# grunwaldlab/krisp

Measured on AMD Instinct MI355X. Metric: k-mers/s sorted+intersected at k=28, higher is better.
Workload: dtype u64

## Files before the change

include/krisp_hip.h:

```cpp
#ifndef KRISP_HIP_H
#define KRISP_HIP_H

#include <stddef.h>
#include <stdint.h>

#ifdef __cplusplus
extern "C" {
#endif

typedef struct kr_ctx kr_ctx;

typedef struct { uint64_t prefix, in_mask, out_mask; } kr_cand;

typedef struct { uint64_t key; uint32_t genome; uint32_t count; } kr_record;

enum {
    KR_OK = 0,
    KR_ERR_HIP = -1,
    KR_ERR_PARAM = -2,
    KR_ERR_CAPACITY = -3,
    KR_ERR_STATE = -4,
    KR_ERR_KEY = -5,
    KR_ERR_HOST = -6
};
// ... 188 lines not shown

int64_t kr_render_records(const kr_record* recs, size_t n, int L, int D, int R, const uint32_t* label_of,
                          size_t n_genomes, const char* const* label_text, size_t n_labels, const uint8_t* label_in,
                          int dot, char** csv, size_t* csv_len, char** align, size_t* align_len);
int64_t kr_render_windows(const uint8_t* rows, size_t n, int L, int D, int R, const uint32_t* cand, const uint32_t* genome,
                          const uint32_t* label_of, size_t n_genomes, const char* const* label_text, size_t n_labels,
                          const uint8_t* label_in, int dot, int rna, char** csv, size_t* csv_len, char** align,
                          size_t* align_len);
void    kr_text_free(void* p);

enum { KR_OPT_SLICE_BASES = 1,
       KR_OPT_GENERIC_INTERSECT = 2,
       KR_OPT_ISECT_FORMAT = 3,
       KR_OPT_ABLATE = 4,
       KR_OPT_WIDE_SLOTS = 5,
       KR_OPT_PLACE_TRIES = 7,
       KR_OPT_ISECT_KERNEL = 8,
       KR_OPT_LANES = 9,
       KR_OPT_LAZY_ORDER = 10,
       KR_OPT_COARSE_REST = 11,
       KR_OPT_COARSE_POOL = 12,
       KR_OPT_JOIN2 = 13,
       KR_OPT_COARSE_ONE_STRAND = 14,
       KR_OPT_WIDE_ORDERED = 6 };
int     kr_set_option(kr_ctx*, int option, int64_t value);

int     kr_sync(kr_ctx*);
int     kr_timer_begin(kr_ctx*);
double  kr_timer_end_ms(kr_ctx*);
int     kr_stage_enable(kr_ctx*, int on);
int     kr_stage_select(kr_ctx*, unsigned stage_mask);
int     kr_stage_reset(kr_ctx*);
double  kr_stage_ms(kr_ctx*, int stage);
int64_t kr_stage_launches(kr_ctx*, int stage);

int64_t kr_debug_fetch(kr_ctx*, int genome_id, int what, void* out, size_t cap_bytes);
int64_t kr_debug_inversions(kr_ctx*, int genome_id);
double  kr_debug_localsort(kr_ctx*, int genome_id, int reps, int mode);
double  kr_debug_intersect(kr_ctx*, const int* genome_ids, int n, const uint8_t* is_ingroup, int reps, int mode);
double  kr_debug_copy_gbps(kr_ctx*, size_t bytes, int reps);
const char* kr_debug_copy_which(kr_ctx*);
int     kr_build_experiments(void);
int     kr_debug_lazy(kr_ctx*, int64_t* out8);
int     kr_debug_isect(kr_ctx*, int64_t* out8);
int     kr_debug_scan(kr_ctx*, int64_t* out8);
int     kr_debug_place(kr_ctx*, double* out8);
int     kr_debug_coarse_pool(kr_ctx*, double* out8);
int     kr_debug_coarse_strand(kr_ctx*, int64_t* out8);
int     kr_debug_comm(kr_ctx*, int64_t* out8);
int     kr_debug_comm_probe(kr_ctx*, size_t bytes, int reps, double* out3);
int64_t kr_debug_cands_selfexchange(kr_ctx*, int apply_filter);
int     kr_debug_comm_hang(kr_ctx*);
int64_t kr_debug_budget_left(kr_ctx*);
int     kr_debug_budget_set(kr_ctx*, int64_t left);
int     kr_debug_info(kr_ctx*, int64_t* out8);

#ifdef __cplusplus
}
#endif
#endif
```

krisp_amd/_native.py:

```python
import ctypes
import os

import numpy as np

HERE = os.path.dirname(os.path.abspath(__file__))
LIB_PATH = os.environ.get("KRISP_HIP_LIB") or os.path.join(HERE, "libkrisp_hip.so")

CAND = np.dtype([("prefix", "<u8"), ("in_mask", "<u8"), ("out_mask", "<u8")])
RECORD = np.dtype([("key", "<u8"), ("genome", "<u4"), ("count", "<u4")])
WIDE_HIT = np.dtype([("cand", "<u4"), ("genome", "<u4"), ("pos", "<u4"), ("strand", "<u4")])
LOC_HIT = np.dtype([("group", "<u4"), ("strand", "<u4"), ("pos", "<u8")])
NEAR_HIT = np.dtype([("target", "<u4"), ("strand", "u1"), ("mismatches", "u1"), ("flank_mismatches", "u1"), ("pad", "u1"),
                     ("pos", "<u8")])
PRODUCT_SITE = np.dtype([("pos", "<u8"), ("entry", "<u4"), ("mismatches", "u1"), ("end_mismatches", "u1"),
                         ("pad", "<u2")])
PRODUCT_HIT = np.dtype([("pos", "<u8"), ("length", "<u4"), ("pair", "<u4"), ("strand", "u1"), ("left_mm", "u1"),
                        ("right_mm", "u1"), ("left_end_mm", "u1"), ("right_end_mm", "u1"), ("pad", "u1", (3,))])
DESIGN_RECORD = np.dtype([("found", "<u4"), ("product_size", "<u4"), ("pair_penalty", "<u4"), ("left_start", "<u2"),
                          ("left_len", "<u2"), ("right_start", "<u2"), ("right_len", "<u2"), ("left_tm", "<i4"), ("right_tm", "<i4"),
                          ("left_gc", "<u2"), ("right_gc", "<u2"), ("left_penalty", "<u4"), ("right_penalty", "<u4"),
                          ("left_self_any", "<i4"), ("left_self_end", "<i4"), ("right_self_any", "<i4"),
                          ("right_self_end", "<i4"), ("pair_any", "<i4"), ("pair_end", "<i4")])
DESIGN_RECORD_HP = np.dtype(DESIGN_RECORD.descr + [("left_hairpin", "<i4"), ("right_hairpin", "<i4")])
PANEL_MEMBER = np.dtype([("position", "<u4"), ("cross_any", "<i4"), ("cross_end", "<i4"), ("dropped", "<u4", (2,))])
# ... 1 lines not shown
GUIDE_RECORD = np.dtype([("found", "<u4"), ("strand", "<u4"), ("start", "<u4"), ("min_mismatches", "<u4"),
                         ("sum_mismatches", "<u4"), ("gc", "<u4"), ("candidates", "<u4"), ("pad", "<u4")])
GUIDE_HIT_RAW = np.dtype([("guide", "<u4"), ("strand", "u1"), ("mismatches", "u1"), ("pam", "u1"), ("pad", "u1"), ("pos", "<u8"),
                          ("columns", "<u8")])
ASSAY_HIT_RAW = np.dtype([("pos", "<u8"), ("length", "<u4"), ("pair", "<u4"), ("strand", "u1"), ("left_mm", "u1"), ("right_mm", "u1"),
                          ("left_end_mm", "u1"), ("right_end_mm", "u1"), ("hit_strand", "u1"), ("hit_mismatches", "u1"),
                          ("hit_pam", "u1"), ("hit_pos", "<u8"), ("columns", "<u8"), ("guide", "<u4"), ("hit", "<u4")])
GUIDE_BULGE_HIT_RAW = np.dtype([("guide", "<u4"), ("strand", "u1"), ("mismatches", "u1"), ("pam", "u1"), ("bulge", "i1"),
                                ("pos", "<u8"), ("columns", "<u8"), ("bulge_column", "<u4"), ("length", "<u4")])
WIDE_DICT_LEFT, WIDE_DICT_RIGHT, WIDE_GROUPS, WIDE_HITS, WIDE_COUNTS, WIDE_SLOT_BITS, WIDE_NGROUPS, WIDE_BATCH_USED, WIDE_LOCATED, WIDE_KEYS_LISTED = 0, 1, 2, 3, 4, 5, 6, 7, 8, 9
WIDE_MAX_K = 1024
WIDE_MAX_FLANK = 256
COMM_ID_BYTES = 128

SOFT_MAP, SOFT_OMIT = 0, 1
OPT_SLICE_BASES, OPT_GENERIC_INTERSECT, OPT_ISECT_FORMAT, OPT_ABLATE, OPT_WIDE_SLOTS, OPT_WIDE_ORDERED, OPT_PLACE_TRIES = 1, 2, 3, 4, 5, 6, 7
OPT_ISECT_KERNEL = 8
OPT_LANES = 9
OPT_LAZY_ORDER = 10
OPT_COARSE_REST = 11
OPT_COARSE_POOL = 12
OPT_JOIN2 = 13
OPT_COARSE_ONE_STRAND = 14
ERR_KEY, ERR_HOST = -5, -6
STRANDS_BOTH, STRANDS_FORWARD, STRANDS_CANONICAL = 0, 1, 2
STAGES = ["pack", "hist8", "reduce8", "scatter1", "hist2", "scan2", "scatter2", "chunks", "localsort",
          "fallback", "intersect", "compact", "collect", "merge", "locate"]
STAGE_KERNELS = {"pack": "k_pack", "hist8": "k_hist8 (wide path: k_hist8w, slices: k_hist8k)", "reduce8": "k_reduce8a+k_reduce8b",
                 "scatter1": "k_scatter1p (wide path: k_scatter1w, slices: k_scatter1kp)",
                 "hist2": "k_hist16 (or k_hist2)", "scan2": "k_hist16_off (or k_scan2)", "scatter2": "k_scatter2",
                 "chunks": "k_chunk_table", "localsort": "k_localsort2",
                 "fallback": "k_seg_merge", "intersect": "k_intersect3 (+ k_intersect for oversized items)",
                 "compact": "k_scan+k_publish_reset+k_gather_items",
                 "collect": "k_collect_count+k_tile_sums+k_scan+k_tile_apply+k_publish+k_collect_emit",
                 "merge": "k_cands_flag+k_scan+k_cands_compact", "locate": "k_wide_locate"}

_c = ctypes
_P = _c.c_void_p
SYMBOLS = [
    ("kr_create", _P, [_c.c_int, _c.c_size_t]),
    ("kr_destroy", None, [_P]),
    ("kr_last_error", _c.c_char_p, [_P]),
    ("kr_set_params", _c.c_int, [_P, _c.c_int, _c.c_int, _c.c_int, _c.c_int, _c.c_size_t]),
    ("kr_set_strands", _c.c_int, [_P, _c.c_int]),
    ("kr_genome_upload", _c.c_int, [_P, _c.c_int, _P, _c.c_size_t]),
    ("kr_genome_sort", _c.c_int, [_P, _c.c_int]),
# ... 825 lines not shown
        v = self.lib.kr_debug_copy_gbps(self.ctx, nbytes, reps)
        if v < 0:
            raise KrispHipError("kr_debug_copy_gbps failed")
        return v

    def mem_info(self):
        o = np.zeros(4, dtype=np.int64)
        self._check(self.lib.kr_mem_info(self.ctx, _ptr(o)), "kr_mem_info")
        return dict(avail=int(o[0]), total=int(o[1]), used=int(o[2]), budget=int(o[3]))

    def debug_comm(self):
        o = np.zeros(8, dtype=np.int64)
        self._check(self.lib.kr_debug_comm(self.ctx, _ptr(o)), "kr_debug_comm")
        return dict(syncs=int(o[0]), p2p=int(o[1]), collectives=int(o[2]), exchange_us=int(o[3]), reduces=int(o[4]),
                    message_entries=int(o[5]))

    def debug_place(self):
        o = np.zeros(8, dtype=np.float64)
        self._check(self.lib.kr_debug_place(self.ctx, _ptr(o)), "kr_debug_place")
        return dict(candidates=int(o[0]), taken=int(o[1]), fastest_ms=[round(float(x), 4) for x in o[2:6]],
                    median_ms=round(float(o[6]), 4), slowest_ms=round(float(o[7]), 4))

    def debug_coarse_strand(self):
        o = np.zeros(8, dtype=np.int64)
        self._check(self.lib.kr_debug_coarse_strand(self.ctx, _ptr(o)), "kr_debug_coarse_strand")
        return dict(partitions=int(o[0]), calls=int(o[1]), rounds_forward=int(o[2]), rounds_reverse=int(o[3]),
                    last_forward=int(o[4]), last_reverse=int(o[5]), on=int(o[6]))

    def debug_coarse_pool(self):
        o = np.zeros(8, dtype=np.float64)
        self._check(self.lib.kr_debug_coarse_pool(self.ctx, _ptr(o)), "kr_debug_coarse_pool")
        return dict(total=int(o[0]), free=int(o[1]), held=int(o[2]), partitions=int(o[3]), searches=int(o[4]),
                    held_ms=[round(float(o[5]), 4), round(float(o[6]), 4)], on=int(o[7]))

    def comm_set_timeout(self, seconds):
        self._check(self.lib.kr_comm_set_timeout(self.ctx, int(seconds)), "kr_comm_set_timeout")

    def debug_comm_hang(self):
        return self._check(self.lib.kr_debug_comm_hang(self.ctx), "kr_debug_comm_hang")

    def cands_selfexchange(self, apply_filter=False):
        return self._check(self.lib.kr_debug_cands_selfexchange(self.ctx, 1 if apply_filter else 0), "kr_debug_cands_selfexchange")

    def comm_probe(self, nbytes=64 << 10, reps=50):
        o = np.zeros(3, dtype=np.float64)
        self._check(self.lib.kr_debug_comm_probe(self.ctx, nbytes, reps, _ptr(o)), "kr_debug_comm_probe")
        return dict(allreduce_sync_us=round(float(o[0]), 2), sendrecv_self_sync_us=round(float(o[1]), 2),
                    bcast_sync_us=round(float(o[2]), 2), message_bytes=int(nbytes))

    def copy_which(self):
# ... 11 lines not shown
```

krisp_amd/csrc/h_core.inc:

```
static thread_local std::string g_last_error;

struct DevBuf {
    void* p = nullptr;
    size_t bytes = 0;
};

struct Slice {
    DevBuf keys, off, chunkstart, chunkdesc, ovf;
    u64 nmax = 0;
    u32 nchunks = 0;
    int64_t count = -1;
    int res = -1;
};

struct Genome {
    int id = -1;
    size_t n_bases = 0;
    u64 nwords = 0;
    u64 nmax = 0;
    DevBuf bases, wkeys;
    DevBuf wlcnt;
    bool wlist = false;
    u32 wlcap = 0;
    std::vector<Slice> sl;
// ... 88 lines not shown
    int join2 = 1;
    u32 j2_grid = 0;
    int j2_occ[9] = {0};
    int64_t j2_launches = 0, j2_full = 0;
    bool j2_full_counted = false;
    int64_t isect_ovf_items = 0, isect_refall = 0;
    int i3_last_T = 0, i3_last_mlog = 0, i3_last_tags = 0, i3_last_ua = 0;
    int64_t isect_ua = 0;
    int fuse_anchor = 1;
    u32 i3_ovf_cap = I3_OVF_CAP;
    int isect_fmt = 0;
    int opt_slice_bases = -1;
    hipEvent_t slice_ready[2] = {nullptr, nullptr};
    bool custom_layout = false;
    bool mixed_alphabets = false;
    int lazy_order = 1;
    bool order_wanted = false;
    int64_t lazy_skipped = 0, lazy_ordered = 0, lazy_touch = 0;
    DevBuf touchdesc, touchovf;
    int coarse_rest = 1;
    int64_t coarse_done = 0, coarse_promoted = 0;
    int coarse_one = 1;
    int64_t one_partitions = 0, one_calls = 0, one_rounds[2] = {0, 0}, one_last[2] = {0, 0};
    DevBuf co_ent;
    int coarse_pool = 1;
    struct PoolBuf { DevBuf buf; double ms; hipEvent_t ev; bool wait; };
    std::vector<PoolBuf> cpool_free;
    int cpool_total = 0;
    int64_t cpool_partitions = 0;
    int64_t cpool_searches = 0;
    size_t place_min_bytes = (size_t)256 << 20;
    DevBuf co_state, co_tab;
    u32 co_tcap = CO_TCAP;
    u32 co_hitcap = 0;
    int co_occ = 0;
    u32 co_grid = 0;
    u32 scan_cap = 0;
    int64_t scan_dbg[3] = {0, 0, 0};
    int slice_route = 1;
    typedef std::vector<DevBuf*> Bufs;
    struct Wide {
        bool on = false;
        int L = 0, D = 0, R = 0, k = 0, omit = 0, W = 0, strands = 0;
        struct DictBufs {
            DevBuf keys, idx, slots;
            DevBuf mzT, mzB;
            int ib = 1, sb = 0, mzlen = 0;
            u32 n = 0, mznb = 0;
            bool canon = false;
            u32 nfull = 0;
            void bufs(Bufs& v) { v.insert(v.end(), {&keys, &idx, &slots, &mzT, &mzB}); }
            Dict view() const {
                Dict d{};
                d.keys = (const u64*)keys.p;
                d.idx = (const u32*)idx.p;
                d.slots = sb && slots.p ? (const uint4*)slots.p : nullptr;
                d.ib = ib;
                d.sb = sb;
// ... 424 lines not shown
        g_last_error = "hipSetDevice failed";
        return nullptr;
    }
    kr_ctx* c = new kr_ctx();
    c->device = device;
    c->budget = hbm_budget_bytes;
    {
        const char* e = getenv("KR_DBG");
        c->dbg = e ? (atoi(e) & 32) : 0;
        const char* e2 = getenv("KR_ISECT_FMT");
        c->isect_fmt = e2 ? (atoi(e2) == 1 ? 1 : (atoi(e2) == 2 ? 2 : 0)) : 0;
        const char* e3 = getenv("KR_SLICE_BASES");
        c->opt_slice_bases = e3 ? std::max(0, std::min(4, atoi(e3))) : -1;
        const char* e16 = getenv("KR_FUSE_ANCHOR");
        c->fuse_anchor = e16 ? atoi(e16) != 0 : 1;
        const char* e15 = getenv("KR_LAZY_ORDER");
        c->lazy_order = e15 ? atoi(e15) != 0 : 1;
        const char* e17 = getenv("KR_COARSE_REST");
        c->coarse_rest = e17 ? atoi(e17) != 0 : 1;
        const char* e21 = getenv("KR_COARSE_POOL");
        c->coarse_pool = e21 ? atoi(e21) != 0 : 1;
        const char* e26 = getenv("KR_COARSE_ONE_STRAND");
        c->coarse_one = e26 ? atoi(e26) != 0 : 1;
        const char* e22 = getenv("KR_PLACE_MIN_BYTES");
        if (e22) c->place_min_bytes = (size_t)std::max(0ll, atoll(e22));
        const char* e18 = getenv("KR_COARSE_TCAP");
        if (e18) c->co_tcap = (u32)std::max(1, std::min((int)CO_TCAP, atoi(e18)));
        const char* e19 = getenv("KR_COARSE_HITCAP");
        if (e19) c->co_hitcap = (u32)std::max(1, atoi(e19));
        const char* e20 = getenv("KR_COARSE_GRID");
        if (e20) c->co_grid = (u32)std::max(0, std::min(65536, atoi(e20)));
        const char* e24 = getenv("KR_JOIN2");
        c->join2 = e24 ? atoi(e24) != 0 : 1;
        const char* e25 = getenv("KR_JOIN2_GRID");
        if (e25) c->j2_grid = (u32)std::max(0, std::min(65536, atoi(e25)));
        const char* e23 = getenv("KR_SCAN_GRID");
        if (e23) c->scan_cap = (u32)std::max(0, std::min(65536, atoi(e23)));
        const char* e13 = getenv("KR_SLICE_ROUTE");
        c->slice_route = e13 ? atoi(e13) != 0 : 1;
        const char* e8 = getenv("KR_PLACE_TRIES");
        c->place_tries = e8 ? std::max(1, std::min(16, atoi(e8))) : 8;
        c->place_tries_set = e8 != nullptr;
        const char* e4 = getenv("KR_WIDE_SLOTS");
        c->wide.use_slots = e4 ? atoi(e4) != 0 : true;
        const char* e7 = getenv("KR_WIDE_SHARE");
        c->wide.use_share = e7 ? atoi(e7) != 0 : true;
        const char* e11 = getenv("KR_WIDE_SPECTRUM");
        c->wide.packed_spectrum = e11 ? atoi(e11) != 0 : true;
        const char* e5 = getenv("KR_WIDE_ORDERED");
        c->wide.ordered = e5 ? atoi(e5) != 0 : false;
// ... 186 lines not shown
        c->place_tries = (int)value;
        c->place_tries_set = true;
        return KR_OK;
    case KR_OPT_WIDE_ORDERED:
        if (value != 0 && value != 1) return fail(c, KR_ERR_PARAM, "KR_OPT_WIDE_ORDERED: 0 or 1");
        c->wide.ordered = value != 0;
        return KR_OK;
    case KR_OPT_LAZY_ORDER:
        if (value != 0 && value != 1) return fail(c, KR_ERR_PARAM, "KR_OPT_LAZY_ORDER: 0 or 1");
        c->lazy_order = (int)value;
        return KR_OK;
    case KR_OPT_COARSE_REST:
        if (value != 0 && value != 1) return fail(c, KR_ERR_PARAM, "KR_OPT_COARSE_REST: 0 or 1");
        c->coarse_rest = (int)value;
        return KR_OK;
    case KR_OPT_COARSE_POOL:
        if (value != 0 && value != 1) return fail(c, KR_ERR_PARAM, "KR_OPT_COARSE_POOL: 0 or 1");
        c->coarse_pool = (int)value;
        return KR_OK;
    case KR_OPT_COARSE_ONE_STRAND:
        if (value != 0 && value != 1) return fail(c, KR_ERR_PARAM, "KR_OPT_COARSE_ONE_STRAND: 0 or 1");
        c->coarse_one = (int)value;
        return KR_OK;
    case KR_OPT_JOIN2:
        if (value != 0 && value != 1) return fail(c, KR_ERR_PARAM, "KR_OPT_JOIN2: 0 or 1");
        c->join2 = (int)value;
        return KR_OK;
    case KR_OPT_ABLATE:
#ifdef KR_ABLATE
        c->dbg = (c->dbg & 32) | ((int)value & ~32);
        return KR_OK;
#else
        return fail(c, KR_ERR_PARAM, "KR_OPT_ABLATE needs a -DKR_ABLATE build");
#endif
    default:
        return fail(c, KR_ERR_PARAM, "unknown option %d", option);
    }
}

int kr_set_strands(kr_ctx* c, int mode) {
    if (!c || !c->have_params) return fail(c, KR_ERR_STATE, "kr_set_params first");
    if (mode < KR_STRANDS_BOTH || mode > KR_STRANDS_CANONICAL) return fail(c, KR_ERR_PARAM, "unknown strand mode %d", mode);
    if (c->wide.on && mode == KR_STRANDS_CANONICAL) return fail(c, KR_ERR_PARAM, "the wide path emits both strands or the forward one");
    if (!c->genomes.empty()) return fail(c, KR_ERR_STATE, "kr_set_strands after genomes were uploaded");
    c->g.strands = mode;
    c->wide.strands = mode;
// ... 1127 lines not shown
```

krisp_amd/csrc/h_intersect.inc:

```
static int64_t intersect_once(kr_ctx* c, const int* ids, int n, const uint8_t* is_in, int apply_filter, bool* redo);

static int64_t cands_merge_device(kr_ctx* c, size_t m, int have_other, int apply_filter);

static inline int fmode(const kr_ctx* c, int apply_filter) { return apply_filter ? (c->mixed_alphabets ? 2 : 1) : 0; }

int kr_set_mixed_alphabets(kr_ctx* c, int on) {
    if (!c) return KR_ERR_PARAM;
    c->mixed_alphabets = on != 0;
    return KR_OK;
}

#define KR_MAX_CANDS 0xFFFFFF00ull
static int cands_fit(kr_ctx* c, uint64_t n, const char* who) {
    if (n < KR_MAX_CANDS) return KR_OK;
    return fail(c, KR_ERR_CAPACITY, "%s: a candidate list of %llu entries exceeds the %llu a list may hold (an intersection that "
                "nothing prunes: give both ingroup and outgroup genomes to one call, or fewer genomes per call)", who,
                (unsigned long long)n, (unsigned long long)KR_MAX_CANDS);
}

static int cands_compact_room(kr_ctx* c, u32 n) {
    const size_t nblk = ((size_t)n + 255) / 256;
    int rc;
    if ((rc = ensure(c, c->flags, (size_t)n * 4))) return rc;
    if ((rc = ensure(c, c->blockcnt, (nblk + 2) * 4))) return rc;
// ... 58 lines not shown
    const u32 nC = (u32)nC64, nblk = (nC + 255) / 256;
    const Geom g = slice_geom(c, 0);
    hipStream_t st = c->stream;
    const u32 hitcap = c->co_hitcap ? c->co_hitcap : (u32)std::min<u64>(2ull * nC + 65536, 0x7FFFFFF0ull);
    if ((rc = ensure(c, c->co_state, (size_t)nC * 4))) return rc;
    if ((rc = ensure(c, c->co_tab, (size_t)(2 * 260 + 256 * CO_ROW) * 4))) return rc;
    if ((rc = cands_compact_room(c, nC))) return rc;
    const size_t ent_bytes = (size_t)2 * nC * sizeof(CoEnt);
    if (one && (rc = ensure(c, c->co_ent, ent_bytes + (size_t)(3 * CS_CLS + 8) * 4))) return rc;
    for (Genome* G : cg) {
        if (G->hitcap < hitcap || !G->hits.p) {
            if ((rc = ensure(c, G->hits, (size_t)hitcap * 8 + 16))) return rc;
        }
        G->hitcap = hitcap;
        G->hits_valid = false;
    }
    if (c->co_occ == 0) {
        int per = 0;
        const hipError_t e = hipOccupancyMaxActiveBlocksPerMultiprocessor(&per, k_coarse_probe<0>, CO_T, 0);
        c->co_occ = (e == hipSuccess && per >= 1) ? per : 1;
        if (hipOccupancyMaxActiveBlocksPerMultiprocessor(&per, k_coarse_probe<1>, CO_T, 0) == hipSuccess && per >= 1)
            c->co_occ = std::min(c->co_occ, per);
    }
    const u32 grid = c->co_grid ? c->co_grid : (u32)(c->co_occ * c->ncu);
    if ((rc = join_lanes(c))) return rc;
    HIPCHK(c, hipMemsetAsync(c->co_state.p, 0, (size_t)nC * 4, st));
    u32 *cb = (u32*)c->co_tab.p, *ust = cb + 260, *rows = cb + 520;
    u32 need = 0;
    CoarsePub pub{};
    pub.n = (int)cg.size();
    CoarseArgs ca{};
    ca.n = (u32)cg.size();
    for (size_t j = 0; j < cg.size(); j++) {
        Genome& G = *cg[j];
        ca.keys[j] = (const u64*)(G.ckeys.p ? G.ckeys.p : G.sl[0].keys.p);
        ca.off[j] = (const u32*)G.sl[0].off.p;
        ca.hits[j] = (u32*)G.hits.p;
        ca.hitcap[j] = hitcap;
        ca.bit[j] = 8u + (u32)j;
        ca.side[j] = is_in[cpos[j]] ? 0u : 4u;
        need |= 1u << (8 + j);
        pub.cnt[j] = (const u32*)G.hits.p;
    }
    {
        StageScope sc(c, KR_ST_INTERSECT, st);
        if (one) {
            const CoStrand S = cs_make(g.L, g.R);
            CoEnt* ents = (CoEnt*)c->co_ent.p;
            u32 *cnt = (u32*)((char*)c->co_ent.p + ent_bytes), *cls = cnt + CS_CLS, *cursor = cls + CS_CLS + 4;
            const u32 cgrid = std::min<u32>((nC + CS_T - 1) / CS_T, (u32)c->ncu);
            HIPCHK(c, hipMemsetAsync(cnt, 0, CS_CLS * 4, st));
            hipLaunchKernelGGL(k_strand_count, dim3(cgrid), dim3(CS_T), 0, st, (const kr_cand*)c->candB.p, nC, S, cnt);
            hipLaunchKernelGGL(k_strand_tables, dim3(1), dim3(CS_CLS), 0, st, (const u32*)cnt, ca, c->co_tcap, cls, cursor, ust, rows,
                               c->mbox + 56);
            hipLaunchKernelGGL(k_strand_fill, dim3(cgrid), dim3(CS_T), 0, st, (const kr_cand*)c->candB.p, nC, S, cursor, ents);
            hipLaunchKernelGGL(k_coarse_probe<1>, dim3(grid), dim3(CO_T), 0, st, ca, (const u32*)cls, (const u32*)ust, (const u32*)rows,
                               (const kr_cand*)c->candB.p, (u32*)c->co_state.p, c->co_tcap, g.pmask, g.LRrel, (const CoEnt*)ents, S);
        } else {
            hipLaunchKernelGGL(k_coarse_tables, dim3(1), dim3(256), 0, st, (const kr_cand*)c->candB.p, nC, ca, c->co_tcap, cb, ust, rows);
            hipLaunchKernelGGL(k_coarse_probe<0>, dim3(grid), dim3(CO_T), 0, st, ca, (const u32*)cb, (const u32*)ust, (const u32*)rows,
                               (const kr_cand*)c->candB.p, (u32*)c->co_state.p, c->co_tcap, g.pmask, g.LRrel, (const CoEnt*)nullptr,
                               CoStrand{});
        }
    }
    for (Genome* G : cg)
        if (G->ckeys.p) G->ckeys_busy = st;
    {
        StageScope sc(c, KR_ST_MERGE, st);
        hipLaunchKernelGGL(k_coarse_flag, dim3(nblk), dim3(256), 0, st, (kr_cand*)c->candB.p, nC, (const u32*)c->co_state.p, need,
                           fmode(c, 1), (u32*)c->flags.p, (u32*)c->blockcnt.p);
        cands_compact_enqueue(c, nC, st, true);
        hipLaunchKernelGGL(k_coarse_publish, dim3(1), dim3(64), 0, st, pub, c->mbox + 32);
    }
    HIPCHK(c, hipStreamSynchronize(st));
    HIPCHK(c, hipGetLastError());
    for (Genome* G : cg) G->ckeys_busy = nullptr;
    if (one) {
        c->one_calls++;
        for (int q = 0; q < 2; q++) {
            c->one_last[q] = ((volatile u32*)c->mbox)[56 + q];
            c->one_rounds[q] += c->one_last[q];
        }
    }
    for (size_t j = 0; j < cg.size(); j++)
        if (((volatile u32*)c->mbox)[32 + j] > hitcap) {
            c->ncand = -1;
            return KR_COARSE_PASS;
        }
    const u32 total = ((volatile u32*)c->mbox)[16];
    cands_compact_adopt(c, total);
    for (Genome* G : cg) G->hits_valid = true;
    c->coarse_done += (int64_t)cg.size();
    {
        int want = 0;
        for (Genome* G : cg) want += !G->ckeys.p && G->partitions >= 2;
        if (want > 0) coarse_pool_grow(c, want);
    }
    return total;
}

int64_t kr_intersect(kr_ctx* c, const int* ids, int n, const uint8_t* is_in, int apply_filter) {
    if (!c || n < 1) return fail(c, KR_ERR_PARAM, "kr_intersect: need at least one genome");
    if (c->custom_layout) return fail(c, KR_ERR_STATE, "kr_intersect: this context sorts by a custom field order (kr_set_field_order)");
    {
// ... 617 lines not shown
```

krisp_amd/csrc/h_misc.inc:

```
double kr_debug_localsort(kr_ctx* c, int id, int reps, int mode) {
    if (!c || mode != 0) return -1.0;
    auto it = c->genomes.find(id);
    if (it != c->genomes.end() && ensure_fine(c, it->second)) return -1.0;
    if (it == c->genomes.end() || !it->second.sorted || it->second.sl.empty()) return -1.0;
    if (ensure_ordered(c, {&it->second}) || finalize(c, {&it->second})) return -1.0;
    Slice& S = it->second.sl[0];
    hipStream_t st = c->stream;
    const u32 grid = std::min<u32>(S.nchunks, (u32)c->ls_grid);
    auto launch = [&]() {
        hipLaunchKernelGGL(k_localsort2, dim3(grid), dim3(LS_THREADS), 0, st, (u64*)S.keys.p, (const u32*)S.off.p,
                           (const uint4*)S.chunkdesc.p, S.nchunks, c->g.b, (u32*)S.ovf.p,
                           (uint4*)((char*)S.ovf.p + 16));
    };
    hipEvent_t a, b;
    (void)hipEventCreate(&a);
    (void)hipEventCreate(&b);
    launch();
    (void)hipEventRecord(a, st);
    for (int r = 0; r < reps; r++) launch();
    (void)hipEventRecord(b, st);
    (void)hipEventSynchronize(b);
    float ms = 0;
    (void)hipEventElapsedTime(&ms, a, b);
    (void)hipEventDestroy(a);
// ... 233 lines not shown
        hi = held ? std::max(hi, G.ckeys_ms) : G.ckeys_ms;
        held++;
    }
    out8[0] = c->cpool_total;
    out8[1] = (double)c->cpool_free.size();
    out8[2] = held;
    out8[3] = (double)c->cpool_partitions;
    out8[4] = (double)c->cpool_searches;
    out8[5] = lo;
    out8[6] = hi;
    out8[7] = c->coarse_pool;
    return KR_OK;
}

int kr_debug_coarse_strand(kr_ctx* c, int64_t* o) {
    if (!c || !o) return KR_ERR_PARAM;
    o[0] = c->one_partitions;
    o[1] = c->one_calls;
    o[2] = c->one_rounds[0];
    o[3] = c->one_rounds[1];
    o[4] = c->one_last[0];
    o[5] = c->one_last[1];
    o[6] = c->coarse_one;
    o[7] = 0;
    return KR_OK;
}

int kr_debug_isect(kr_ctx* c, int64_t* o) {
    if (!c || !o) return KR_ERR_PARAM;
    o[0] = c->isect_ovf_items;
    o[1] = c->isect_refall;
    o[2] = c->i3_last_T;
    o[3] = c->i3_last_mlog;
    o[4] = c->i3_last_tags;
    o[5] = lanes_used(c);
    o[6] = c->j2_launches;
    o[7] = c->j2_full;
    return KR_OK;
}

int kr_debug_scan(kr_ctx* c, int64_t* o) {
    if (!c || !o) return KR_ERR_PARAM;
    o[0] = c->scan_dbg[0];
    o[1] = c->scan_dbg[1];
    o[2] = c->scan_cap;
    o[3] = c->scan_dbg[2];
    o[4] = o[5] = o[6] = o[7] = 0;
// ... 55 lines not shown
```

krisp_amd/csrc/k_coarse.inc:

```

#include "co_units.inc"

#define CO_T 1024
#define CO_SLOT_LOG 13
#define CO_SLOTS (1u << CO_SLOT_LOG)
#define CO_BM_LOG 17
#define CO_QCAP 2048
#define CO_TCAP 6144
#define CO_EMPTY 0xFFFFFFFFu
#define CO_UNROLL 4
#define CO_ITER (2u * CO_T * CO_UNROLL)
#define CO_HB 1024
#define CO_MAXG 24
#define CO_ROW (2 * CO_MAXG)

struct CoarseArgs {
    const u64* keys[CO_MAXG];
    const u32* off[CO_MAXG];
    u32* hits[CO_MAXG];
    u32 hitcap[CO_MAXG];
    u32 bit[CO_MAXG];
    u32 side[CO_MAXG];
    u32 n;
};
// ... 50 lines not shown
    const u32 len = above ? (u32)__builtin_ctzll(above) + 1u : 64u - lane;
    u32 r0 = 0;
    if (head && active) r0 = atomicAdd(&h[c], len);
    return (u32)__shfl((int)r0, (int)leader) + (lane - leader);
}

__global__ __launch_bounds__(CS_T) void k_strand_count(const kr_cand* __restrict__ cands, u32 n, CoStrand S, u32* __restrict__ cnt) {
    __shared__ u32 h[CS_CLS];
    if (threadIdx.x < CS_CLS) h[threadIdx.x] = 0;
    __syncthreads();
    for (u32 i0 = blockIdx.x * CS_T; i0 < n; i0 += gridDim.x * CS_T) {
        const u32 i = i0 + threadIdx.x;
        const bool on = i < n;
        const u64 P = cands[on ? i : n - 1].prefix;
        (void)co_run_add(h, 2 * cs_class_fwd(S, P), on);
        if (on) atomicAdd(&h[2 * cs_class_rev(S, P) + 1], 1u);
    }
    __syncthreads();
    for (u32 t = threadIdx.x; t < CS_CLS; t += CS_T)
        if (h[t]) atomicAdd(&cnt[t], h[t]);
}

__device__ __forceinline__ u32 co_rounds(u32 nc, u32 tcap) { return nc / tcap + (nc % tcap ? 1u : 0u); }
__global__ __launch_bounds__(CS_CLS) void k_strand_tables(const u32* __restrict__ cnt, CoarseArgs A, u32 tcap, u32* __restrict__ cls,
                                                          u32* __restrict__ cursor, u32* __restrict__ ust, u32* rows,
                                                          u32* __restrict__ host_rounds) {
    __shared__ u32 waves[17];
    const u32 t = threadIdx.x;
    u32 total;
    const u32 ex = block_excl_scan(cnt[t], waves, total);
    cls[t] = ex;
    cursor[t] = ex;
    if (t == 0) cls[CS_CLS] = total;
    if (t < 4 * A.n) A.hits[t >> 2][t & 3u] = 0;
    u32 units = 0, rf = 0, rr = 0;
    if (t < 256) {
        u32* row = rows + t * CO_ROW;
        for (u32 j = 0; j < A.n; j++) {
            row[2 * j] = A.off[j][t];
            row[2 * j + 1] = A.off[j][t + 1];
        }
        rf = co_rounds(cnt[2 * t], tcap);
        rr = co_rounds(cnt[2 * t + 1], tcap);
        units = co_byte_units((rf + rr) * tcap, tcap, row, A.n);
        if (co_row_chunks(row, A.n) == 0) rf = rr = 0;
    }
    const u32 ux = block_excl_scan(units, waves, total);
    if (t < 256) ust[t] = ux;
    if (t == 0) ust[256] = total;
    (void)block_excl_scan(rf, waves, total);
    if (t == 0) host_rounds[0] = total;
    (void)block_excl_scan(rr, waves, total);
    if (t == 0) host_rounds[1] = total;
}

__global__ __launch_bounds__(CS_T) void k_strand_fill(const kr_cand* __restrict__ cands, u32 n, CoStrand S, u32* __restrict__ cursor,
                                                     CoEnt* __restrict__ ents) {
    __shared__ u32 h[CS_CLS], base[CS_CLS];
    if (threadIdx.x < CS_CLS) h[threadIdx.x] = 0;
    __syncthreads();
    for (u32 i0 = blockIdx.x * CS_T; i0 < n; i0 += gridDim.x * CS_T) {
        const u32 i = i0 + threadIdx.x;
        const bool on = i < n;
        const u64 P = cands[on ? i : n - 1].prefix;
        (void)co_run_add(h, 2 * cs_class_fwd(S, P), on);
        if (on) atomicAdd(&h[2 * cs_class_rev(S, P) + 1], 1u);
    }
    __syncthreads();
    for (u32 t = threadIdx.x; t < CS_CLS; t += CS_T) {
        base[t] = h[t] ? atomicAdd(&cursor[t], h[t]) : 0u;
        h[t] = 0;
    }
    __syncthreads();
    for (u32 i0 = blockIdx.x * CS_T; i0 < n; i0 += gridDim.x * CS_T) {
        const u32 i = i0 + threadIdx.x;
        const bool on = i < n;
        const u64 P = cands[on ? i : n - 1].prefix;
        const u32 cf = 2 * cs_class_fwd(S, P), cr = 2 * cs_class_rev(S, P) + 1;
        const u32 rank = co_run_add(h, cf, on);
        if (!on) continue;
        CoEnt e;
        e.ci = i;
        e.pad = 0;
        e.pat = P;
        ents[base[cf] + rank] = e;
        e.pat = cs_pattern_rev(S, P);
        ents[base[cr] + atomicAdd(&h[cr], 1u)] = e;
    }
}

template <int OS>
__device__ __forceinline__ void co_lookup(u64 key, u64 pmask, int LR, const u32* slots, u32 c0, const kr_cand* __restrict__ cands,
                                          u32* __restrict__ state, u32 orbits, u32 side_shift, u64* s_hit, u32* s_nhit,
                                          u32* __restrict__ hits, u64* __restrict__ hitkeys, u32 hitcap,
                                          const CoEnt* __restrict__ ents, bool rev, const CoStrand& S) {
    const u64 pre = key & pmask;
    const u32 h = co_hash(pre);
    const u32 tag = h & 0x7FFFFu;
    u32 s = h >> (32 - CO_SLOT_LOG);
    for (u32 w = slots[s]; w != CO_EMPTY; w = slots[s]) {
        if ((w & 0x7FFFFu) == tag) {
            u32 ci = c0 + (w >> 19);
            if ((OS ? ents[ci].pat : cands[ci].prefix) == pre) {
                if (OS) {
                    ci = ents[ci].ci;
                    if (rev) key = cs_rev_key(S, key);
                }
                const u32 at0 = atomicAdd(s_nhit, 1u);
                if (at0 < CO_HB) s_hit[at0] = key;
// ... 181 lines not shown
            __syncthreads();
            const u32 hb = s_hbase;
            for (u32 i = threadIdx.x; i < m; i += CO_T)
                if (hb + i < hitcap) hitkeys[hb + i] = s_hit[i];
        }
        __syncthreads();
        if (++u >= u1) return true;
        if (ahead) adopt(un);
        else {
            new_byte();
            cold = true;
        }
        return false;
    };

    u32x4 va[CO_UNROLL], vb[CO_UNROLL];
    new_byte();
    for (;;) {
        if (step(va, vb)) break;
        if (step(vb, va)) break;
    }
}

__global__ void k_coarse_flag(kr_cand* __restrict__ cur, u32 n, const u32* __restrict__ state, u32 need, int mode,
                              u32* __restrict__ flags, u32* __restrict__ blockcnt) {
    __shared__ u32 waves[17];
    const u32 i = blockIdx.x * blockDim.x + threadIdx.x;
    bool keep = false;
    if (i < n) {
        const u32 st = state[i];
        keep = (st & need) == need;
        if (keep) {
            kr_cand c = cur[i];
            c.in_mask |= st & 15u;
            c.out_mask |= (st >> 4) & 15u;
            keep = passes_filter(c.in_mask, c.out_mask, 1, mode);
            if (keep) cur[i] = c;
        }
        flags[i] = keep ? 1u : 0u;
    }
    u32 tot;
    block_compact(keep, waves, tot);
    if (threadIdx.x == 0) blockcnt[blockIdx.x] = tot;
}

struct CoarsePub { const u32* cnt[CO_MAXG]; int n; };
// ... 50 lines not shown
```

Baseline: 133.1 billion.

## Add single shared-memory table probe for both strands with bloom-bitmap prefilter

Adds a one-table coarse probe kernel that stores forward and reverse-strand candidate patterns together in one 16-bit-slot shared-memory hash table. A two-bit bloom bitmap filters keys before they are queued for exact lookup. Each key stream is now read once per unit instead of once per strand round, and most hash probes on non-matching keys are skipped. The cost is a larger shared-memory footprint, a per-unit queue that falls back to a direct scan when it overflows, and extra table and bitmap build work. The new path is on by default and can be disabled with an option or environment variable.

```diff
diff --git a/include/krisp_hip.h b/include/krisp_hip.h
--- a/include/krisp_hip.h
+++ b/include/krisp_hip.h
@@ -234,6 +234,7 @@
        KR_OPT_COARSE_POOL = 12,
        KR_OPT_JOIN2 = 13,
        KR_OPT_COARSE_ONE_STRAND = 14,
+       KR_OPT_COARSE_ONE_TABLE = 15,
        KR_OPT_WIDE_ORDERED = 6 };
 int     kr_set_option(kr_ctx*, int option, int64_t value);
 
@@ -258,7 +259,7 @@
 int     kr_debug_scan(kr_ctx*, int64_t* out8);
 int     kr_debug_place(kr_ctx*, double* out8);
 int     kr_debug_coarse_pool(kr_ctx*, double* out8);
-int     kr_debug_coarse_strand(kr_ctx*, int64_t* out8);
+int     kr_debug_coarse_strand(kr_ctx*, int64_t* out12);
 int     kr_debug_comm(kr_ctx*, int64_t* out8);
 int     kr_debug_comm_probe(kr_ctx*, size_t bytes, int reps, double* out3);
 int64_t kr_debug_cands_selfexchange(kr_ctx*, int apply_filter);
diff --git a/krisp_amd/_native.py b/krisp_amd/_native.py
--- a/krisp_amd/_native.py
+++ b/krisp_amd/_native.py
@@ -47,6 +47,7 @@
 OPT_COARSE_POOL = 12
 OPT_JOIN2 = 13
 OPT_COARSE_ONE_STRAND = 14
+OPT_COARSE_ONE_TABLE = 15
 ERR_KEY, ERR_HOST = -5, -6
 STRANDS_BOTH, STRANDS_FORWARD, STRANDS_CANONICAL = 0, 1, 2
 STAGES = ["pack", "hist8", "reduce8", "scatter1", "hist2", "scan2", "scatter2", "chunks", "localsort",
@@ -918,10 +919,11 @@
                     median_ms=round(float(o[6]), 4), slowest_ms=round(float(o[7]), 4))
 
     def debug_coarse_strand(self):
-        o = np.zeros(8, dtype=np.int64)
+        o = np.zeros(12, dtype=np.int64)
         self._check(self.lib.kr_debug_coarse_strand(self.ctx, _ptr(o)), "kr_debug_coarse_strand")
         return dict(partitions=int(o[0]), calls=int(o[1]), rounds_forward=int(o[2]), rounds_reverse=int(o[3]),
-                    last_forward=int(o[4]), last_reverse=int(o[5]), on=int(o[6]))
+                    last_forward=int(o[4]), last_reverse=int(o[5]), on=int(o[6]), one_table=int(o[7]),
+                    one_table_calls=int(o[8]), one_table_rounds=int(o[9]), one_table_last=int(o[10]))
 
     def debug_coarse_pool(self):
         o = np.zeros(8, dtype=np.float64)
diff --git a/krisp_amd/csrc/co_onetable.inc b/krisp_amd/csrc/co_onetable.inc
--- /dev/null
+++ b/krisp_amd/csrc/co_onetable.inc
@@ -0,0 +1,40 @@
+#include <stdint.h>
+
+#define CO1_SLOT_LOG 14
+#define CO1_SLOTS (1u << CO1_SLOT_LOG)
+#define CO1_TCAP 12288u
+#define CO1_EMPTY 0xFFFFu
+#define CO1_BM_LOG 18
+
+__host__ __device__ inline uint32_t co1_hash(uint64_t pat, uint32_t reading) {
+    const uint32_t lo = (uint32_t)pat;
+    const uint32_t h = ((uint32_t)(pat >> 32) ^ ((lo >> 16) | (lo << 16))) * 0x85EBCA6Bu;
+    return reading ? ~h : h;
+}
+__host__ __device__ inline uint32_t co1_slot(uint32_t h) { return h >> (32 - CO1_SLOT_LOG); }
+__host__ __device__ inline uint32_t co1_tag(uint32_t h) { return (h >> 10) & 3u; }
+__host__ __device__ inline uint32_t co1_word(uint32_t idx, uint32_t h) { return (idx << 2) | co1_tag(h); }
+__host__ __device__ inline uint32_t co1_bm_word(uint32_t h) { return h >> (37 - CO1_BM_LOG); }
+__host__ __device__ inline uint32_t co1_bm_bits(uint32_t h) { return (1u << ((h >> 5) & 31u)) | (1u << (h & 31u)); }
+__host__ __device__ inline uint32_t co1_bm_both(uint32_t word, uint32_t h) { return (word >> ((h >> 5) & 31u)) & (word >> (h & 31u)); }
+__host__ __device__ inline bool co1_bm_pass(uint32_t word, uint32_t h) { return (co1_bm_both(word, h) & 1u) != 0; }
+
+#define CO1_NONE 0xFFFFFFFFu
+template <class Ent>
+__host__ __device__ inline uint32_t co1_find(const uint16_t* slots, const Ent* ents, uint64_t pre, uint32_t reading, uint32_t h) {
+    const uint32_t tag = co1_tag(h);
+    uint32_t s = co1_slot(h);
+    for (uint32_t w = slots[s]; w != CO1_EMPTY; w = slots[s]) {
+        if ((w & 3u) == tag) {
+            const uint32_t idx = w >> 2;
+            if (ents[idx].pat == pre && ents[idx].pad == reading) return idx;
+        }
+        s = (s + 1) & (CO1_SLOTS - 1);
+    }
+    return CO1_NONE;
+}
+
+__host__ __device__ inline uint32_t co1_rounds(uint32_t nf, uint32_t nr, uint32_t tcap1) {
+    const uint32_t n = nf + nr;
+    return n / tcap1 + (n % tcap1 ? 1u : 0u);
+}
diff --git a/krisp_amd/csrc/h_core.inc b/krisp_amd/csrc/h_core.inc
--- a/krisp_amd/csrc/h_core.inc
+++ b/krisp_amd/csrc/h_core.inc
@@ -134,6 +134,8 @@
     int64_t coarse_done = 0, coarse_promoted = 0;
     int coarse_one = 1;
     int64_t one_partitions = 0, one_calls = 0, one_rounds[2] = {0, 0}, one_last[2] = {0, 0};
+    int coarse_one_table = 1;
+    int64_t one1_calls = 0, one1_rounds = 0, one1_last = 0;
     DevBuf co_ent;
     int coarse_pool = 1;
     struct PoolBuf { DevBuf buf; double ms; hipEvent_t ev; bool wait; };
@@ -144,8 +146,10 @@
     size_t place_min_bytes = (size_t)256 << 20;
     DevBuf co_state, co_tab;
     u32 co_tcap = CO_TCAP;
+    u32 co_tcap1 = CO1_TCAP;
     u32 co_hitcap = 0;
     int co_occ = 0;
+    int co_occ1 = 0;
     u32 co_grid = 0;
     u32 scan_cap = 0;
     int64_t scan_dbg[3] = {0, 0, 0};
@@ -616,10 +620,13 @@
         c->coarse_pool = e21 ? atoi(e21) != 0 : 1;
         const char* e26 = getenv("KR_COARSE_ONE_STRAND");
         c->coarse_one = e26 ? atoi(e26) != 0 : 1;
+        const char* e27 = getenv("KR_COARSE_ONE_TABLE");
+        c->coarse_one_table = e27 ? atoi(e27) != 0 : 1;
         const char* e22 = getenv("KR_PLACE_MIN_BYTES");
         if (e22) c->place_min_bytes = (size_t)std::max(0ll, atoll(e22));
         const char* e18 = getenv("KR_COARSE_TCAP");
         if (e18) c->co_tcap = (u32)std::max(1, std::min((int)CO_TCAP, atoi(e18)));
+        if (e18) c->co_tcap1 = (u32)std::max(1, std::min((int)CO1_TCAP, atoi(e18)));
         const char* e19 = getenv("KR_COARSE_HITCAP");
         if (e19) c->co_hitcap = (u32)std::max(1, atoi(e19));
         const char* e20 = getenv("KR_COARSE_GRID");
@@ -852,6 +859,10 @@
         if (value != 0 && value != 1) return fail(c, KR_ERR_PARAM, "KR_OPT_COARSE_ONE_STRAND: 0 or 1");
         c->coarse_one = (int)value;
         return KR_OK;
+    case KR_OPT_COARSE_ONE_TABLE:
+        if (value != 0 && value != 1) return fail(c, KR_ERR_PARAM, "KR_OPT_COARSE_ONE_TABLE: 0 or 1");
+        c->coarse_one_table = (int)value;
+        return KR_OK;
     case KR_OPT_JOIN2:
         if (value != 0 && value != 1) return fail(c, KR_ERR_PARAM, "KR_OPT_JOIN2: 0 or 1");
         c->join2 = (int)value;
diff --git a/krisp_amd/csrc/h_intersect.inc b/krisp_amd/csrc/h_intersect.inc
--- a/krisp_amd/csrc/h_intersect.inc
+++ b/krisp_amd/csrc/h_intersect.inc
@@ -104,7 +104,13 @@
         if (hipOccupancyMaxActiveBlocksPerMultiprocessor(&per, k_coarse_probe<1>, CO_T, 0) == hipSuccess && per >= 1)
             c->co_occ = std::min(c->co_occ, per);
     }
-    const u32 grid = c->co_grid ? c->co_grid : (u32)(c->co_occ * c->ncu);
+    const bool one_table = one && c->coarse_one_table;
+    if (one_table && c->co_occ1 == 0) {
+        int per = 0;
+        const hipError_t e = hipOccupancyMaxActiveBlocksPerMultiprocessor(&per, k_coarse_probe1, CO_T, 0);
+        c->co_occ1 = (e == hipSuccess && per >= 1) ? per : 1;
+    }
+    const u32 grid = c->co_grid ? c->co_grid : (u32)((one_table ? c->co_occ1 : c->co_occ) * c->ncu);
     if ((rc = join_lanes(c))) return rc;
     HIPCHK(c, hipMemsetAsync(c->co_state.p, 0, (size_t)nC * 4, st));
     u32 *cb = (u32*)c->co_tab.p, *ust = cb + 260, *rows = cb + 520;
@@ -133,11 +139,16 @@
             const u32 cgrid = std::min<u32>((nC + CS_T - 1) / CS_T, (u32)c->ncu);
             HIPCHK(c, hipMemsetAsync(cnt, 0, CS_CLS * 4, st));
             hipLaunchKernelGGL(k_strand_count, dim3(cgrid), dim3(CS_T), 0, st, (const kr_cand*)c->candB.p, nC, S, cnt);
-            hipLaunchKernelGGL(k_strand_tables, dim3(1), dim3(CS_CLS), 0, st, (const u32*)cnt, ca, c->co_tcap, cls, cursor, ust, rows,
-                               c->mbox + 56);
+            hipLaunchKernelGGL(k_strand_tables, dim3(1), dim3(CS_CLS), 0, st, (const u32*)cnt, ca, c->co_tcap,
+                               one_table ? c->co_tcap1 : 0u, cls, cursor, ust, rows, c->mbox + 56);
             hipLaunchKernelGGL(k_strand_fill, dim3(cgrid), dim3(CS_T), 0, st, (const kr_cand*)c->candB.p, nC, S, cursor, ents);
-            hipLaunchKernelGGL(k_coarse_probe<1>, dim3(grid), dim3(CO_T), 0, st, ca, (const u32*)cls, (const u32*)ust, (const u32*)rows,
-                               (const kr_cand*)c->candB.p, (u32*)c->co_state.p, c->co_tcap, g.pmask, g.LRrel, (const CoEnt*)ents, S);
+            if (one_table)
+                hipLaunchKernelGGL(k_coarse_probe1, dim3(grid), dim3(CO_T), 0, st, ca, (const u32*)cls, (const u32*)ust, (const u32*)rows,
+                                   (u32*)c->co_state.p, c->co_tcap1, g.pmask, g.LRrel, (const CoEnt*)ents, S);
+            else
+                hipLaunchKernelGGL(k_coarse_probe<1>, dim3(grid), dim3(CO_T), 0, st, ca, (const u32*)cls, (const u32*)ust,
+                                   (const u32*)rows, (const kr_cand*)c->candB.p, (u32*)c->co_state.p, c->co_tcap, g.pmask, g.LRrel,
+                                   (const CoEnt*)ents, S);
         } else {
             hipLaunchKernelGGL(k_coarse_tables, dim3(1), dim3(256), 0, st, (const kr_cand*)c->candB.p, nC, ca, c->co_tcap, cb, ust, rows);
             hipLaunchKernelGGL(k_coarse_probe<0>, dim3(grid), dim3(CO_T), 0, st, ca, (const u32*)cb, (const u32*)ust, (const u32*)rows,
@@ -162,6 +173,11 @@
         for (int q = 0; q < 2; q++) {
             c->one_last[q] = ((volatile u32*)c->mbox)[56 + q];
             c->one_rounds[q] += c->one_last[q];
+        }
+        if (one_table) {
+            c->one1_calls++;
+            c->one1_last = ((volatile u32*)c->mbox)[58];
+            c->one1_rounds += c->one1_last;
         }
     }
     for (size_t j = 0; j < cg.size(); j++)
diff --git a/krisp_amd/csrc/h_misc.inc b/krisp_amd/csrc/h_misc.inc
--- a/krisp_amd/csrc/h_misc.inc
+++ b/krisp_amd/csrc/h_misc.inc
@@ -279,7 +279,11 @@
     o[4] = c->one_last[0];
     o[5] = c->one_last[1];
     o[6] = c->coarse_one;
-    o[7] = 0;
+    o[7] = c->coarse_one_table;
+    o[8] = c->one1_calls;
+    o[9] = c->one1_rounds;
+    o[10] = c->one1_last;
+    o[11] = 0;
     return KR_OK;
 }
 
diff --git a/krisp_amd/csrc/k_coarse.inc b/krisp_amd/csrc/k_coarse.inc
--- a/krisp_amd/csrc/k_coarse.inc
+++ b/krisp_amd/csrc/k_coarse.inc
@@ -1,5 +1,6 @@
 
 #include "co_units.inc"
+#include "co_onetable.inc"
 
 #define CO_T 1024
 #define CO_SLOT_LOG 13
@@ -96,9 +97,9 @@
 }
 
 __device__ __forceinline__ u32 co_rounds(u32 nc, u32 tcap) { return nc / tcap + (nc % tcap ? 1u : 0u); }
-__global__ __launch_bounds__(CS_CLS) void k_strand_tables(const u32* __restrict__ cnt, CoarseArgs A, u32 tcap, u32* __restrict__ cls,
-                                                          u32* __restrict__ cursor, u32* __restrict__ ust, u32* rows,
-                                                          u32* __restrict__ host_rounds) {
+__global__ __launch_bounds__(CS_CLS) void k_strand_tables(const u32* __restrict__ cnt, CoarseArgs A, u32 tcap, u32 tcap1,
+                                                          u32* __restrict__ cls, u32* __restrict__ cursor, u32* __restrict__ ust,
+                                                          u32* rows, u32* __restrict__ host_rounds) {
     __shared__ u32 waves[17];
     const u32 t = threadIdx.x;
     u32 total;
@@ -107,7 +108,7 @@
     cursor[t] = ex;
     if (t == 0) cls[CS_CLS] = total;
     if (t < 4 * A.n) A.hits[t >> 2][t & 3u] = 0;
-    u32 units = 0, rf = 0, rr = 0;
+    u32 units = 0, rf = 0, rr = 0, r1 = 0;
     if (t < 256) {
         u32* row = rows + t * CO_ROW;
         for (u32 j = 0; j < A.n; j++) {
@@ -116,8 +117,11 @@
         }
         rf = co_rounds(cnt[2 * t], tcap);
         rr = co_rounds(cnt[2 * t + 1], tcap);
-        units = co_byte_units((rf + rr) * tcap, tcap, row, A.n);
-        if (co_row_chunks(row, A.n) == 0) rf = rr = 0;
+        if (tcap1) {
+            r1 = co1_rounds(cnt[2 * t], cnt[2 * t + 1], tcap1);
+            units = co_byte_units(cnt[2 * t] + cnt[2 * t + 1], tcap1, row, A.n);
+        } else units = co_byte_units((rf + rr) * tcap, tcap, row, A.n);
+        if (co_row_chunks(row, A.n) == 0) rf = rr = r1 = 0;
     }
     const u32 ux = block_excl_scan(units, waves, total);
     if (t < 256) ust[t] = ux;
@@ -126,6 +130,8 @@
     if (t == 0) host_rounds[0] = total;
     (void)block_excl_scan(rr, waves, total);
     if (t == 0) host_rounds[1] = total;
+    (void)block_excl_scan(r1, waves, total);
+    if (t == 0) host_rounds[2] = total;
 }
 
 __global__ __launch_bounds__(CS_T) void k_strand_fill(const kr_cand* __restrict__ cands, u32 n, CoStrand S, u32* __restrict__ cursor,
@@ -159,6 +165,7 @@
         e.pat = P;
         ents[base[cf] + rank] = e;
         e.pat = cs_pattern_rev(S, P);
+        e.pad = 1;
         ents[base[cr] + atomicAdd(&h[cr], 1u)] = e;
     }
 }
@@ -386,6 +393,243 @@
     }
 }
 
+#define CO1_QCAP 1536
+#define CO1_BMW (1u << (CO1_BM_LOG - 5))
+
+template <u32 RD>
+__device__ __forceinline__ bool co1_lookup(u64 key, u64 mask, int LR, const unsigned short* slots, const u32* bitmap, u32 c0,
+                                           const CoEnt* __restrict__ ents, u32* __restrict__ state, u32 orbits, u32 side_shift,
+                                           const CoStrand& S, u64& rec) {
+    const u64 pre = key & mask;
+    const u32 h = co1_hash(pre, RD);
+    if (!co1_bm_pass(bitmap[co1_bm_word(h)], h)) return false;
+    const u32 idx = co1_find(slots, ents + c0, pre, RD, h);
+    if (idx == CO1_NONE) return false;
+    rec = RD ? cs_rev_key(S, key) : key;
+    const u32 bb = (u32)(rec >> (62 - 2 * LR)) & 3u;
+    atomicOr(&state[ents[c0 + idx].ci], orbits | (1u << (side_shift + bb)));
+    return true;
+}
+
+__global__ __launch_bounds__(CO_T, 8) void k_coarse_probe1(CoarseArgs A, const u32* __restrict__ cls, const u32* __restrict__ ust,
+                                                        const u32* __restrict__ rows, u32* __restrict__ state, u32 tcap1, u64 pmask,
+                                                        int LR, const CoEnt* __restrict__ ents, CoStrand S) {
+    __shared__ u32 slots32[CO1_SLOTS / 2];
+    __shared__ u32 bitmap[CO1_BMW];
+    __shared__ u32 s_ust[257];
+    __shared__ u32 s_bnd[CO_ROW];
+    __shared__ u64 s_q[CO1_QCAP];
+    __shared__ u32 s_nhit, s_hbase, s_qn;
+    const unsigned short* slots = reinterpret_cast<const unsigned short*>(slots32);
+    if (threadIdx.x == 0) { s_nhit = 0; s_qn = 0; }
+    for (u32 t = threadIdx.x; t <= 256; t += CO_T) s_ust[t] = ust[t];
+    __syncthreads();
+    const u32 G = A.n;
+    const u32 U = s_ust[256];
+    const u32 u0 = (u32)(((u64)blockIdx.x * U) / gridDim.x), u1 = (u32)(((u64)(blockIdx.x + 1) * U) / gridDim.x);
+    if (u0 >= u1) return;
+    const u32 lane = threadIdx.x & 63u;
+    const u64 mask_rc = S.mask_rc;
+    u32 u = u0, t = 0, ust_t = 0, ust_t1 = 0, k0 = 0, k1 = 0, p0 = 0, c0 = 0;
+    u32 cur_t = ~0u, cur_r = ~0u;
+    u32 nhit_before = 0;
+    const u64* __restrict__ kp = nullptr;
+    u32* __restrict__ hits = nullptr;
+    u64* __restrict__ hitkeys = nullptr;
+    u32 hitcap = 0, orbits = 0, side_shift = 0;
+    bool cold = true;
+
+    auto adopt = [&](const CoUnit& un) {
+        const u32 g = un.genome, r = un.round;
+        k0 = un.k0;
+        k1 = un.k1;
+        p0 = k0 & ~1u;
+        kp = A.keys[g];
+        hits = A.hits[g];
+        hitkeys = (u64*)(hits + 4);
+        hitcap = A.hitcap[g];
+        orbits = 1u << A.bit[g];
+        side_shift = A.side[g];
+        if (t != cur_t || r != cur_r) {
+            cur_t = t;
+            cur_r = r;
+            for (u32 i = threadIdx.x; i < CO1_SLOTS / 2; i += CO_T) slots32[i] = 0xFFFFFFFFu;
+            for (u32 i = threadIdx.x; i < CO1_BMW; i += CO_T) bitmap[i] = 0;
+            __syncthreads();
+            const u32 e1 = cls[2 * t + 2];
+            c0 = cls[2 * t] + r * tcap1;
+            const u32 c1 = e1 - c0 > tcap1 ? c0 + tcap1 : e1;
+            for (u32 i = c0 + threadIdx.x; i < c1; i += CO_T) {
+                const CoEnt e = ents[i];
+                const u32 h = co1_hash(e.pat, e.pad);
+                const u32 word = co1_word(i - c0, h);
+                u32 s = co1_slot(h);
+                for (;;) {
+                    const u32 sh = (s & 1u) * 16u;
+                    const u32 old = __hip_atomic_load(&slots32[s >> 1], __ATOMIC_RELAXED, __HIP_MEMORY_SCOPE_WORKGROUP);
+                    if (((old >> sh) & 0xFFFFu) != CO1_EMPTY) { s = (s + 1) & (CO1_SLOTS - 1); continue; }
+                    const u32 nw = (old & ~(0xFFFFu << sh)) | (word << sh);
+                    if (atomicCAS(&slots32[s >> 1], old, nw) == old) break;
+                }
+                atomicOr(&bitmap[co1_bm_word(h)], co1_bm_bits(h));
+            }
+            __syncthreads();
+        }
+    };
+    auto uniform = [](CoUnit un) {
+        un.round = CO_RFL(un.round); un.genome = CO_RFL(un.genome); un.chunk = CO_RFL(un.chunk);
+        un.k0 = CO_RFL(un.k0); un.k1 = CO_RFL(un.k1);
+        return un;
+    };
+    auto new_byte = [&]() {
+        t = CO_RFL(co_unit_byte(s_ust, u));
+        ust_t = CO_RFL(s_ust[t]);
+        ust_t1 = CO_RFL(s_ust[t + 1]);
+        if (threadIdx.x < 2 * G) s_bnd[threadIdx.x] = rows[t * CO_ROW + threadIdx.x];
+        __syncthreads();
+        adopt(uniform(co_unit_decode(u - ust_t, s_bnd, G)));
+    };
+    auto step = [&](u32x4 (&V)[CO_UNROLL], u32x4 (&NV)[CO_UNROLL]) -> bool {
+        const bool last = k1 - p0 <= CO_ITER;
+        bool ahead = false;
+        CoUnit un = {};
+        const u64* __restrict__ nkp = kp;
+        u32 np0 = p0 + CO_ITER, na0 = k0 & ~1u, nk1 = k1;
+        if (last) {
+            np0 = na0;
+            nk1 = 0;
+            if (u + 1 < u1 && u + 1 < ust_t1) {
+                un = uniform(co_unit_decode(u + 1 - ust_t, s_bnd, G));
+                nkp = A.keys[un.genome];
+                np0 = na0 = un.k0 & ~1u;
+                nk1 = un.k1;
+                ahead = true;
+            }
+        }
+        if (cold) co_load(V, kp, p0, p0, k1);
+        cold = false;
+        co_load(NV, nkp, np0, na0, nk1);
+        __builtin_amdgcn_sched_barrier(0);
+        const int hi = (int)(k1 - p0) - 2 * (int)threadIdx.x;
+        const bool front = p0 < k0 && threadIdx.x == 0;
+#pragma unroll
+        for (int q0 = 0; q0 < CO_UNROLL; q0 += 2) {
+            u32 hh[8], ww[8];
+            u64 bal[4];
+            u32 wq = 0;
+#pragma unroll
+            for (int j = 0; j < 4; j++) {
+                const int q = q0 + (j >> 1), e = j & 1;
+                const u64 key = e ? ((u64)V[q].w << 32 | V[q].z) : ((u64)V[q].y << 32 | V[q].x);
+                hh[2 * j] = co1_hash(key & pmask, 0u);
+                hh[2 * j + 1] = co1_hash(key & mask_rc, 1u);
+            }
+#pragma unroll
+            for (int j = 0; j < 8; j++) ww[j] = bitmap[co1_bm_word(hh[j])];
+#pragma unroll
+            for (int j = 0; j < 4; j++) {
+                const int q = q0 + (j >> 1), e = j & 1;
+                const bool inr = (2 * q * (int)CO_T + e < hi) & !(q == 0 && e == 0 && front);
+                const bool mine = (((co1_bm_both(ww[2 * j], hh[2 * j]) | co1_bm_both(ww[2 * j + 1], hh[2 * j + 1])) & 1u) != 0) & inr;
+                bal[j] = __builtin_amdgcn_ballot_w64(mine);
+                wq += (u32)__popcll(bal[j]);
+            }
+            if (wq) {
+                u32 qb = 0;
+                if (lane == 0) qb = atomicAdd(&s_qn, wq);
+                qb = CO_RFL(qb);
+#pragma unroll
+                for (int j = 0; j < 4; j++) {
+                    const int q = q0 + (j >> 1), e = j & 1;
+                    const u64 b = bal[j];
+                    if (b) {
+                        const u64 key = e ? ((u64)V[q].w << 32 | V[q].z) : ((u64)V[q].y << 32 | V[q].x);
+                        const u32 qa = qb + __builtin_amdgcn_mbcnt_hi((u32)(b >> 32), __builtin_amdgcn_mbcnt_lo((u32)b, 0u));
+                        if (((b >> lane) & 1ull) && qa < CO1_QCAP) s_q[qa] = key;
+                        qb += (u32)__popcll(b);
+                    }
+                }
+            }
+        }
+        if (!last) { p0 += CO_ITER; return false; }
+        __syncthreads();
+        u64 rec[4] = {0, 0, 0, 0};
+        bool on[4] = {false, false, false, false};
+        const u32 qn = s_qn;
+        if (qn <= CO1_QCAP) {
+#pragma unroll
+            for (int j = 0; j < 2; j++) {
+                const u32 i = threadIdx.x + (u32)j * CO_T;
+                if (i < qn) {
+                    const u64 key = s_q[i];
+                    on[2 * j] = co1_lookup<0>(key, pmask, LR, slots, bitmap, c0, ents, state, orbits, side_shift, S, rec[2 * j]);
+                    on[2 * j + 1] = co1_lookup<1>(key, mask_rc, LR, slots, bitmap, c0, ents, state, orbits, side_shift, S, rec[2 * j + 1]);
+                }
+            }
+        } else {
+            const u32 a0 = k0 & ~1u;
+            for (u32 p = a0 + 2 * threadIdx.x; p < k1; p += 2 * CO_T) {
+                const u32x4 w = *reinterpret_cast<const u32x4*>(kp + p);
+#pragma unroll
+                for (int e = 0; e < 2; e++) {
+                    const u64 key = e ? ((u64)w.w << 32 | w.z) : ((u64)w.y << 32 | w.x);
+                    if (p + e < k0 || p + e >= k1) continue;
+                    u64 r2[2];
+                    bool o2[2];
+                    o2[0] = co1_lookup<0>(key, pmask, LR, slots, bitmap, c0, ents, state, orbits, side_shift, S, r2[0]);
+                    o2[1] = co1_lookup<1>(key, mask_rc, LR, slots, bitmap, c0, ents, state, orbits, side_shift, S, r2[1]);
+#pragma unroll
+                    for (int j = 0; j < 2; j++)
+                        if (o2[j]) {
+                            const u32 pos = atomicAdd(hits, 1u);
+                            if (pos < hitcap) hitkeys[pos] = r2[j];
+                        }
+                }
+            }
+        }
+        u32 at[4], wn = 0;
+#pragma unroll
+        for (int j = 0; j < 4; j++) {
+            const u64 bal = __builtin_amdgcn_ballot_w64(on[j]);
+            at[j] = wn + __builtin_amdgcn_mbcnt_hi((u32)(bal >> 32), __builtin_amdgcn_mbcnt_lo((u32)bal, 0u));
+            wn += (u32)__popcll(bal);
+        }
+        u32 wb = 0;
+        if (wn) {
+            if (lane == 0) wb = atomicAdd(&s_nhit, wn);
+            wb = CO_RFL(wb);
+        }
+        __syncthreads();
+        const u32 nhit = s_nhit, m = nhit - nhit_before;
+        if (threadIdx.x == 0) {
+            s_qn = 0;
+            if (m) s_hbase = atomicAdd(hits, m);
+        }
+        __syncthreads();
+        if (m) {
+            const u32 hb = s_hbase + (wb - nhit_before);
+#pragma unroll
+            for (int j = 0; j < 4; j++)
+                if (on[j] && hb + at[j] < hitcap) hitkeys[hb + at[j]] = rec[j];
+        }
+        nhit_before = nhit;
+        if (++u >= u1) return true;
+        if (ahead) adopt(un);
+        else {
+            new_byte();
+            cold = true;
+        }
+        return false;
+    };
+
+    u32x4 va[CO_UNROLL], vb[CO_UNROLL];
+    new_byte();
+    for (;;) {
+        if (step(va, vb)) break;
+        if (step(vb, va)) break;
+    }
+}
+
 __global__ void k_coarse_flag(kr_cand* __restrict__ cur, u32 n, const u32* __restrict__ state, u32 need, int mode,
                               u32* __restrict__ flags, u32* __restrict__ blockcnt) {
     __shared__ u32 waves[17];
```

New measurement: 133.1 billion, median of 2. Within noise of the previous version (+0.0%).
